# Sartor02/libMultiRobotPlanning

Hardware: AMD Instinct MI355X
Metric: low_level_node_expansions_per_sec (higher is better)
Workload: dtype int32

## Files before the change

### libmultirobotplanning_amd/csrc/ll_jobs.h

```cpp
#ifndef MRP_LL_JOBS_H
#define MRP_LL_JOBS_H

namespace mrp {

__host__ __device__ inline uint32_t ldsBytes(uint32_t pathBytes, bool bg) { return ct::windowBytes(bg) + pathBytes; }

DEVI uint32_t storeLoad(const uint16_t* p) {
#ifdef MRP_LL_STORE_ACQUIRE_FENCE
  return *p;
#else
  return __hip_atomic_load(p, __ATOMIC_RELAXED, __HIP_MEMORY_SCOPE_AGENT);
#endif
}

DEVI uint32_t hostLoad32(const uint32_t* p) { return __hip_atomic_load(p, __ATOMIC_RELAXED, __HIP_MEMORY_SCOPE_SYSTEM); }
DEVI void hostStore32(uint32_t* p, uint32_t v) { __hip_atomic_store(p, v, __ATOMIC_RELAXED, __HIP_MEMORY_SCOPE_SYSTEM); }

DEVI void stageConstraints(const uint32_t* consHost, uint32_t vcOff, uint32_t nVc, uint32_t nEc, uint32_t* consLocal,
                           const uint32_t*& vc, const uint32_t*& ec) {
  const uint32_t* src = consHost + vcOff;
  const uint32_t nWords = nVc + nEc;
  if (nWords <= kConsLocalWords) {
    for (uint32_t i = threadIdx.x; i < nWords; i += 64) consLocal[i] = hostLoad32(src + i);
    vc = consLocal;
  } else {
    __builtin_amdgcn_fence(__ATOMIC_ACQUIRE, "");
    vc = src;
  }
  ec = vc + nVc;
}

__device__ __attribute__((noinline)) bool stageConstraintSet(const DevJob* job, const uint32_t* cons, uint32_t* store, uint32_t stride,
                                                             uint32_t slots, uint32_t* consLocal) {
  const uint32_t nVc = rfl(job->n_vc), nEc = rfl(job->n_ec), dimx = rfl(job->dimx), dimy = rfl(job->dimy);
  const uint32_t baseP1 = rfl(job->pad_[0]), baseCounts = rfl(job->pad_[1]), resP1 = rfl(job->pad_[2]);
  const uint32_t* added = cons + rfl(job->vc_off);
  stride = rfl(stride); slots = rfl(slots);
  const uint32_t bVc = baseP1 ? (baseCounts & 0xFFFFu) : 0u, bEc = baseP1 ? (baseCounts >> 16) : 0u;
  const uint32_t nWords = nVc + nEc;
  if (store == nullptr || baseP1 > slots || resP1 > slots || bVc > nVc || bEc > nEc || nVc > kConsLocalWords ||
      nEc > kConsLocalWords || nWords > kConsLocalWords || nWords > stride)
    return false;
  const uint32_t aVc = nVc - bVc;
  const uint32_t cells = dimx * dimy;
  const uint32_t* base = store + (size_t)(baseP1 ? baseP1 - 1u : 0u) * stride;
  uint32_t* out = store + (size_t)(resP1 ? resP1 - 1u : 0u) * stride;
  for (uint32_t i = threadIdx.x; i < nWords; i += 64) {
    uint32_t w;
    if (i < nVc) {
      if (i < bVc) {
        w = __hip_atomic_load(base + i, __ATOMIC_RELAXED, __HIP_MEMORY_SCOPE_AGENT);
        if ((w & 0xFFu) >= dimx || ((w >> 8) & 0xFFu) >= dimy) w = 0xFFFFFFFFu;
      } else {
        w = hostLoad32(added + (i - bVc));
      }
    } else {
      const uint32_t k = i - nVc;
      if (k < bEc) {
        w = __hip_atomic_load(base + bVc + k, __ATOMIC_RELAXED, __HIP_MEMORY_SCOPE_AGENT);
        if (((w >> 3) & 0xFFFFu) >= cells) w = 0xFFFFFFFFu;
      } else {
        w = hostLoad32(added + aVc + (k - bEc));
      }
    }
    consLocal[i] = w;
    if (resP1) __hip_atomic_store(out + i, w, __ATOMIC_RELAXED, __HIP_MEMORY_SCOPE_AGENT);
  }
  return true;
}

template <bool UNI = false>
DEVI void fillCtx(Ctx& c, const DevJob& J, const uint32_t* maps, volatile uint32_t* debug) {
  auto u = [](uint32_t v) { return UNI ? rfl(v) : v; };
  c.dimx = u(J.dimx); c.dimy = u(J.dimy); c.wpr = u(J.words_per_row);
  c.gx = u(J.gx); c.gy = u(J.gy); c.sx = u(J.sx); c.sy = u(J.sy);
  c.lastGoal = (int32_t)u((uint32_t)J.last_goal_constraint);
  c.w = __builtin_bit_cast(float, u(__builtin_bit_cast(uint32_t, J.w)));
  c.nVc = u(J.n_vc); c.nEc = u(J.n_ec);
  c.obst = maps + u(J.map_word_off);
  c.nAgentsPad = u(J.n_agents_pad); c.tPad = u(J.t_pad);
  c.maxExp = UNI ? (int64_t)rfl64((uint64_t)J.max_expansions) : J.max_expansions;
  c.debug = debug;
}

DEVI void putCJob(uint8_t* smem, const ct::CJob& cj) {
  auto w32 = (__attribute__((address_space(3))) uint32_t*)((wv::Lds)smem + ct::oJob);
  const uint32_t* src = (const uint32_t*)&cj;
#pragma unroll
  for (uint32_t q = 0; q < sizeof(ct::CJob) / 4; ++q) w32[q] = src[q];
}
DEVI ct::CRes getCRes(uint8_t* smem) {
  auto r32 = (__attribute__((address_space(3))) const uint32_t*)((wv::Lds)smem + ct::oRes);
  ct::CRes cr;
  cr.status = (int32_t)rfl(r32[0]); cr.cost = (int32_t)rfl(r32[1]); cr.fmin = (int32_t)rfl(r32[2]);
  cr.nStates = (int32_t)rfl(r32[3]); cr.expanded = rfl(r32[4]); cr.nodes = rfl(r32[5]);
  return cr;
}
DEVI uint32_t narrowOpenCap(const LaunchParams& P) { return P.lds_nodes / 2u < ct::kCap ? P.lds_nodes / 2u : ct::kCap; }
DEVI uint32_t narrowMaxT(const LaunchParams& P) {
  return P.lds_rows >= 3u && P.lds_rows - 2u < ct::kMaxT ? P.lds_rows - 2u : ct::kMaxT;
}
DEVI uint32_t clampMaxExp(int64_t maxExp) {
  return maxExp < 0 ? 0xFFFFFFFFu : (maxExp > 0xFFFFFFFEll ? 0xFFFFFFFEu : (uint32_t)maxExp);
}

DEVI uint8_t* cutHeaps(Mem<TierHbm>& g, uint8_t* p, uint32_t cap) {
  g.open = (Mem<TierHbm>::PE)(p + 8);          p += (size_t)cap * 8 + 16;
  g.focal = (Mem<TierHbm>::PE)(p + 8);         p += (size_t)cap * 8 + 16;
  g.aux = (Mem<TierHbm>::PE)(p + 8);           p += (size_t)cap * 8 + 16;
  g.capNodes = cap; g.capHeap = cap;
  return p;
}
DEVI Mem<TierHbm> cutArena(const LaunchParams& P, uint8_t* arenaSlot) {
  Mem<TierHbm> g = {};
  g.nodes = (Mem<TierHbm>::PN32)arenaSlot;
  g.bits = (Mem<TierHbm>::P32)cutHeaps(g, arenaSlot + slot::nodeBytes(P.arena_nodes), P.arena_nodes);
  g.capRows = P.arena_rows; g.rowWords = P.arena_row_words;
  return g;
}
template <class Geo>
DEVI bool compactFits(uint32_t arenaNodes, uint32_t rows, bool bg) {
  return slot::nodeBytes(arenaNodes) >= Geo::parentBytes(rows) + (bg ? Geo::bitsBytes(rows) : 0u);
}
template <class Geo = ct::Narrow>
DEVI ct::CJob baseCJob(const LaunchParams& P, const DevJob& J, uint8_t* arenaSlot, uint16_t* outPath, uint32_t rows = 0) {
  ct::CJob cj;
  cj.dimx = J.dimx; cj.dimy = J.dimy; cj.w = J.w; cj.obstWords = J.words_per_row;
  cj.obst = (uint64_t)(P.maps + J.map_word_off);
  cj.maxExp = clampMaxExp(J.max_expansions);
  cj.openCap = narrowOpenCap(P); cj.maxT = narrowMaxT(P); cj.taNoGoal = 0; cj.rows = 0;
  cj.parentTab = (uint64_t)arenaSlot; cj.bitsG = (uint64_t)(arenaSlot + Geo::parentBytes(rows)); cj.outPath = (uint64_t)outPath;
  return cj;
}

enum : int { kTiersAll = 0, kTiersFront = 1, kTiersHeavy = 2 };

template <int TIERS>
DEVI bool idTableInLds(const LaunchParams& P, uint32_t pathBytes) {
  return TIERS != kTiersHeavy && P.lds_nodes != 0 && pathBytes <= P.lds_paths_bytes;
}

DEVI bool frontHandsOver(const LaunchParams& P, const DevJob& J) {
  return (J.ctx_flags & kCtxHeavy) != 0 || P.lds_nodes == 0 || J.dimx > 32u || J.dimy > 32u || J.n_agents_pad > 128u || J.n_ec > 64u;
}

DEVI void clearIdTable(uint16_t* dst, uint32_t pathBytes) {
  uint32_t* d32 = (uint32_t*)dst;
  for (uint32_t i = threadIdx.x; i < pathBytes / 4; i += 64) d32[i] = 0xFFFFFFFFu;
#ifdef MRP_LL_STORE_ACQUIRE_FENCE
  __builtin_amdgcn_fence(__ATOMIC_ACQUIRE, "agent");
  asm volatile("s_waitcnt vmcnt(0)" ::: "memory");
#endif
  __syncthreads();
}
DEVI void loadIdChunk(const uint32_t* ids, uint32_t a0, uint32_t nCtx, const uint16_t* store, uint32_t stride, uint32_t slots,
                      uint32_t& idL, uint32_t& lenL) {
  const uint32_t lane = threadIdx.x;
  idL = kNoStoreSlot; lenL = 0;
  if (a0 + lane < nCtx) idL = hostLoad32(ids + a0 + lane);
  if (idL < slots) lenL = storeLoad(store + (size_t)idL * stride);
  if (lenL > stride - 1) lenL = stride - 1;
}
DEVI void buildIdTableInArena(uint16_t* dst, const uint32_t* ids, uint32_t nCtx, uint32_t tPad, uint32_t nAgentsPad,
                              const uint16_t* store, uint32_t stride, uint32_t slots) {
  const uint32_t lane = threadIdx.x;
  clearIdTable(dst, tPad * nAgentsPad * 2);
  for (uint32_t a0 = 0; a0 < nCtx; a0 += 64) {
    uint32_t idL, lenA;
    loadIdChunk(ids, a0, nCtx, store, stride, slots, idL, lenA);
    const uint16_t* slotA = store + (size_t)(idL < slots ? idL : 0) * stride + 1;
    const bool hasA = idL < slots && lenA != 0;
    for (uint32_t t0 = 0; t0 < tPad; t0 += 8) {
      uint32_t v[8];
#pragma unroll
      for (uint32_t u = 0; u < 8; ++u) {
        const uint32_t t = t0 + u;
        v[u] = kEmptyCell;
        if (hasA && t < tPad) v[u] = storeLoad(slotA + (t < lenA ? t : lenA - 1));
      }
#pragma unroll
      for (uint32_t u = 0; u < 8; ++u)
        if (hasA && t0 + u < tPad) dst[(t0 + u) * nAgentsPad + a0 + lane] = (uint16_t)v[u];
    }
  }
}

template <int TIERS>
DEVI bool stageFocalTable(const LaunchParams& P, const DevJob& J, uint8_t* ldsPaths, uint8_t* pathsArena, Ctx& c) {
  constexpr bool kTableMayBeInLds = TIERS != kTiersHeavy;
  const uint32_t lane = threadIdx.x;
  const uint32_t pathBytes = c.tPad * c.nAgentsPad * 2;
  const uint32_t* psrc = (const uint32_t*)(P.paths + J.path_off);
  c.pathsLds = nullptr;
  if (pathBytes != 0 && (J.ctx_flags & kCtxById)) {
    const bool inLds = idTableInLds<TIERS>(P, pathBytes);
    if (!inLds && pathBytes > P.arena_paths_bytes) return false;
    uint16_t* dst = inLds ? (uint16_t*)ldsPaths : (uint16_t*)pathsArena;
    const uint32_t* ids = P.cons + J.path_off;
    const uint32_t nCtx = J.n_ctx;
    if (!inLds) {
      buildIdTableInArena(dst, ids, nCtx, c.tPad, c.nAgentsPad, P.path_store, P.path_store_stride, P.path_store_slots);
    } else {
      clearIdTable(dst, pathBytes);
      for (uint32_t a0 = 0; a0 < nCtx; a0 += 64) {
        uint32_t idL, lenL;
        loadIdChunk(ids, a0, nCtx, P.path_store, P.path_store_stride, P.path_store_slots, idL, lenL);
        const uint32_t nHere = nCtx - a0 < 64 ? nCtx - a0 : 64;
        for (uint32_t t0 = 0; t0 < c.tPad; t0 += 64) {
          const uint32_t t = t0 + lane;
          for (uint32_t q0 = 0; q0 < nHere; q0 += 8) {
            uint32_t v[8];
            bool has[8];
#pragma unroll
            for (uint32_t u = 0; u < 8; ++u) {
              uint32_t id = kNoStoreSlot, len = 0;
              if (q0 + u < nHere) {
                id = __builtin_amdgcn_readlane(idL, q0 + u);
                len = __builtin_amdgcn_readlane(lenL, q0 + u);
              }
              has[u] = id < P.path_store_slots && len != 0 && t < c.tPad;
              v[u] = kEmptyCell;
              if (has[u]) v[u] = storeLoad(P.path_store + (size_t)id * P.path_store_stride + 1 + (t < len ? t : len - 1));
            }
#pragma unroll
            for (uint32_t u = 0; u < 8; ++u)
              if (has[u]) dst[t * c.nAgentsPad + a0 + q0 + u] = (uint16_t)v[u];
          }
        }
      }
    }
    c.paths = dst;
    if (inLds) c.pathsLds = (__attribute__((address_space(3))) const uint16_t*)ldsPaths;
  } else if (pathBytes == 0) {
    c.paths = nullptr;
  } else if (kTableMayBeInLds && P.lds_nodes != 0 && pathBytes <= P.lds_paths_bytes) {
    uint32_t* dst = (uint32_t*)ldsPaths;
    for (uint32_t i = lane; i < pathBytes / 4; i += 64) dst[i] = hostLoad32(psrc + i);
    c.paths = (const uint16_t*)ldsPaths;
    c.pathsLds = (__attribute__((address_space(3))) const uint16_t*)ldsPaths;
  } else if (pathBytes <= P.arena_paths_bytes) {
    uint32_t* dst = (uint32_t*)pathsArena;
    for (uint32_t i = lane; i < pathBytes / 4; i += 64) dst[i] = hostLoad32(psrc + i);
    c.paths = (const uint16_t*)pathsArena;
  } else {
    __builtin_amdgcn_fence(__ATOMIC_ACQUIRE, "");
    c.paths = P.paths + J.path_off;
  }
  return true;
}

template <bool EPS, bool BG, int TIERS, bool TH = false>
DEVI bool compactAttempt(const LaunchParams& P, const DevJob& J, uint8_t* smem, uint8_t* arenaSlot, const Ctx& c, DevResult& res,
                         uint16_t* outPath, SState& s, int& rc, const uint16_t* heur = nullptr) {
  static_assert(!TH || (!BG && TIERS == kTiersAll), "the table form exists for the mixed kernels' narrow tier");
  typedef typename std::conditional<TIERS == kTiersHeavy, ct::Wide, ct::Narrow>::type Geo;
  uint32_t geoRows = Geo::kRows;
  if (TIERS == kTiersHeavy) {
    const uint64_t room = slot::nodeBytes(P.arena_nodes) / (1024u + ct::kRowBytes);
    geoRows = (uint32_t)(room < P.arena_rows ? room : P.arena_rows) & ~63u;
  }
  const bool compactOk = !(TIERS == kTiersAll && (J.ctx_flags & kCtxHeavy) != 0) && P.lds_nodes != 0 && c.dimx <= 32u &&
                         c.dimy <= 32u && c.nAgentsPad <= 128u && c.nEc <= 64u && geoRows >= 64u &&
                         compactFits<Geo>(P.arena_nodes, geoRows, BG) &&
                         (!TH || P.lds_paths_bytes >= 2048u + (EPS && c.pathsLds != nullptr ? c.tPad * c.nAgentsPad * 2u : 0u));
  bool done = false;
  if (compactOk) {
    ct::CJob cj = baseCJob<Geo>(P, J, arenaSlot, outPath, geoRows);
    cj.obstWords = c.wpr;
    cj.sx = c.sx; cj.sy = c.sy; cj.gx = c.gx; cj.gy = c.gy;
    cj.lastGoal = c.lastGoal;
    cj.nVc = c.nVc; cj.nEc = c.nEc;
    cj.nAgentsPad = EPS ? c.nAgentsPad : 0u; cj.tPad = c.tPad;
    cj.rows = geoRows;
    if (TIERS == kTiersHeavy) {
      cj.openCap = Geo::kCap;
      cj.maxT = Geo::kMaxT < geoRows - 2u ? Geo::kMaxT : geoRows - 2u;
    }
    cj.vc = (uint64_t)c.vc; cj.ec = (uint64_t)c.ec;
    cj.pathsG = (uint64_t)c.paths;
    if constexpr (TH) cj.bitsG = (uint64_t)heur;
    putCJob(smem, cj);
    const bool tableInLds = !EPS || c.nAgentsPad == 0u || c.pathsLds != nullptr;
#ifndef MRP_LL_TRACE
    const uint64_t tl0 = __builtin_amdgcn_s_memrealtime();
#endif
    int32_t crc;
    if constexpr (TH && !EPS)
      crc = ct::compactSearch<false, true, false, ct::Narrow, true>((wv::Lds)smem);
    else if constexpr (TH)
      crc = tableInLds ? ct::compactSearch<true, true, false, ct::Narrow, true>((wv::Lds)smem)
                       : ct::compactSearch<true, false, false, ct::Narrow, true>((wv::Lds)smem);
    else if constexpr (TIERS == kTiersHeavy)
      crc = ct::compactSearch<EPS, false, BG, ct::Wide>((wv::Lds)smem);
    else
      crc = tableInLds ? ct::compactSearch<EPS, true, BG>((wv::Lds)smem) : ct::compactSearch<EPS, false, BG>((wv::Lds)smem);
    const ct::CRes cr = getCRes(smem);
#ifndef MRP_LL_TRACE
    res.prof[TIERS == kTiersHeavy ? 2 : 0] = (uint32_t)(__builtin_amdgcn_s_memrealtime() - tl0);
    res.prof[TIERS == kTiersHeavy ? 3 : 1] = cr.expanded;
#endif
#ifdef MRP_CT_PROF
    {
      auto r32 = (__attribute__((address_space(3))) const uint32_t*)((wv::Lds)smem + ct::oRes + 32u);
      for (uint32_t q = 0; q < 8; ++q) res.prof[q] = rfl(r32[q]);
    }
#endif
    if (crc != ct::C_OVERFLOW) {
      rc = crc;
      res.cost = cr.cost; res.fmin = cr.fmin; res.n_states = cr.nStates;
      s.expansions = cr.expanded; s.nNodes = cr.nodes;
      done = true;
      if (TIERS == kTiersHeavy) res.tier = 2;
    } else {
#ifndef MRP_LL_TRACE
      res.prof[6] = cr.expanded;
      res.prof[7] = 1;
#endif
    }
  }
  return done;
}

template <bool EPS, bool BG, int TIERS, bool TH = false>
DEVI int arenaAttempt(const LaunchParams& P, uint8_t* smem, uint8_t* arenaSlot, const Ctx& c, DevResult& res, uint16_t* outPath,
                      SState& s, const uint16_t* heur = nullptr, uint32_t heurStride = 0) {
  typedef typename std::conditional<TIERS == kTiersHeavy, ct::Wide, ct::Narrow>::type Geo;
  int rc;
  const Mem<TierHbm> g = cutArena(P, arenaSlot);
  Mem<TierHyb> gh = viewAs<TierHyb>(g);
  {
    const uint32_t area = Geo::windowBytes(BG) - ct::oOpen;
#ifdef MRP_LL_TOPS_EQUAL
    const uint32_t perO = (area / 3u) & ~15u, perF = perO, perA = perO;
#else
    const uint32_t perO = (area / 2u) & ~15u, perF = (area * 5u / 16u) & ~15u, perA = (area - perO - perF) & ~15u;
#endif
    auto tops = [&](uint32_t per) {
      uint32_t n = per >= 32u ? ((per - 8u) / 8u) : 0u;
      if (n > 4095u) n = 4095u;
      n = n ? ((n - 1u) | 1u) : 0u;
      return P.lds_nodes == 0 ? 0u : n;
    };
    auto l8 = (__attribute__((address_space(3))) uint8_t*)smem + ct::oOpen;
    gh.open = HybPtr{(__attribute__((address_space(3))) uint64_t*)(l8 + 8), (uint64_t*)g.open, tops(perO)};
    gh.focal = HybPtr{(__attribute__((address_space(3))) uint64_t*)(l8 + perO + 8), (uint64_t*)g.focal, tops(perF)};
    gh.aux = HybPtr{(__attribute__((address_space(3))) uint64_t*)(l8 + perO + perF + 8), (uint64_t*)g.aux, tops(perA)};
  }
  const bool xyEntries = P.arena_nodes <= 65536u;
  Mem<TierHybXy> ghx = viewAs<TierHybXy>(gh);
  res.tier = 1;
  __syncthreads();
  if constexpr (TH) {
    if (xyEntries)
      initSearch<TierHybXy, EPS, true>(ghx, s, c, heur, heurStride);
    else
      initSearch<TierHyb, EPS, true>(gh, s, c, heur, heurStride);
  } else if (xyEntries)
    initSearch<TierHybXy, EPS>(ghx, s, c);
  else
    initSearch<TierHyb, EPS>(gh, s, c);
  __syncthreads();
#ifndef MRP_LL_TRACE
  const uint64_t th0 = __builtin_amdgcn_s_memrealtime();
#endif
  if constexpr (TH) {
    if (xyEntries)
      rc = runSearch<TierHybXy, EPS, true>(ghx, s, c, res, outPath, heur, heurStride);
    else
      rc = runSearch<TierHyb, EPS, true>(gh, s, c, res, outPath, heur, heurStride);
  } else if (xyEntries)
    rc = runSearch<TierHybXy, EPS>(ghx, s, c, res, outPath);
  else
    rc = runSearch<TierHyb, EPS>(gh, s, c, res, outPath);
#ifndef MRP_LL_TRACE
  if (TIERS != kTiersHeavy) {
    res.prof[2] = (uint32_t)(__builtin_amdgcn_s_memrealtime() - th0);
    res.prof[3] = (uint32_t)s.expansions;
  }
#endif
  return rc;
}

template <bool EPS, bool BG, int TIERS>
DEVI bool runJob(const LaunchParams& P, const DevJob& J, uint8_t* smem, uint8_t* arenaSlot, DevResult& res,
                 uint16_t* outPath) {
  typedef typename std::conditional<TIERS == kTiersHeavy, ct::Wide, ct::Narrow>::type Geo;
  if (TIERS == kTiersFront && frontHandsOver(P, J)) return true;
  Ctx c;
  fillCtx(c, J, P.maps, P.debug);
  uint32_t* consLocal = slot::consCopy(arenaSlot, P.arena_scratch_off, P.out_stride);
  if ((J.pad_[0] | J.pad_[2]) != 0u) {
    c.vc = consLocal;
    c.ec = consLocal + c.nVc;
  } else {
    stageConstraints(P.cons, J.vc_off, c.nVc, c.nEc, consLocal, c.vc, c.ec);
  }
  if (!stageFocalTable<TIERS>(P, J, smem + Geo::windowBytes(BG), slot::pathsCopy(arenaSlot, P.arena_scratch_off, P.out_stride), c)) {
    res.status = ST_BAD; res.expanded = 0; res.nodes_created = 0;
    return false;
  }
  __syncthreads();
  SState s;
  int rc = ST_BAD;
  res.tier = 0;
  if (!compactAttempt<EPS, BG, TIERS>(P, J, smem, arenaSlot, c, res, outPath, s, rc)) {
    if constexpr (TIERS == kTiersFront)
      return true;
    else
      rc = arenaAttempt<EPS, BG, TIERS>(P, smem, arenaSlot, c, res, outPath, s);
  }
  if (rc == RUN_MIGRATE_NODES) rc = ST_CAP_NODES;
  if (rc == RUN_MIGRATE_ROWS) rc = ST_CAP_HORIZON;
  res.status = rc;
  res.expanded = s.expansions;
  res.nodes_created = s.nNodes;
  return false;
}

template <bool EPS>
__device__ __attribute__((noinline)) void runJobTableH(const DevJob* Jp, DevResult* out, uint8_t* smem, uint8_t* arenaSlot,
                                                       const uint32_t* maps, const uint32_t* consHost, const uint16_t* pathsHost,
                                                       uint32_t scratchOff, uint32_t outStride, uint32_t arenaNodes,
                                                       uint32_t arenaRows, uint32_t arenaRowWords, uint32_t arenaPathsBytes,
                                                       uint32_t ldsNodes, uint32_t ldsPathsBytes) {
  LaunchParams P = {};
  P.maps = (const uint32_t*)rfl64((uint64_t)maps);
  P.cons = (const uint32_t*)rfl64((uint64_t)consHost);
  P.paths = (const uint16_t*)rfl64((uint64_t)pathsHost);
  P.arena_scratch_off = rfl(scratchOff); P.out_stride = rfl(outStride);
  P.arena_nodes = rfl(arenaNodes); P.arena_rows = rfl(arenaRows); P.arena_row_words = rfl(arenaRowWords);
  P.arena_paths_bytes = rfl(arenaPathsBytes);
  P.lds_nodes = rfl(ldsNodes); P.lds_paths_bytes = rfl(ldsPathsBytes);
  smem = (uint8_t*)rfl64((uint64_t)smem);
  arenaSlot = (uint8_t*)rfl64((uint64_t)arenaSlot);
  DevJob J;
  for (uint32_t q = 0; q < sizeof(DevJob) / 4; ++q) ((uint32_t*)&J)[q] = rfl(((const uint32_t*)Jp)[q]);
  J.ctx_flags &= ~kCtxById;
  DevResult res = {};
  Ctx c;
  fillCtx(c, J, P.maps, nullptr);
  if (!EPS) { c.nAgentsPad = 0; c.tPad = 0; }
  uint16_t* outPath = slot::outPath(arenaSlot, P.arena_scratch_off, P.out_stride);
  stageConstraints(P.cons, J.vc_off, c.nVc, c.nEc, slot::consCopy(arenaSlot, P.arena_scratch_off, P.out_stride), c.vc, c.ec);
  {
    LaunchParams Pst = P;
    Pst.lds_paths_bytes = P.lds_paths_bytes >= 2048u ? P.lds_paths_bytes - 2048u : 0u;
    stageFocalTable<kTiersAll>(Pst, J, smem + ct::Narrow::windowBytes(false), slot::pathsCopy(arenaSlot, P.arena_scratch_off, P.out_stride), c);
  }
  __syncthreads();
  const uint16_t* heur = (const uint16_t*)(P.maps + J.heur_off);
  const uint32_t heurStride = (c.dimx <= 32u && c.dimy <= 32u) ? 32u : c.dimx;
  const bool startInMap = c.sx < c.dimx && c.sy < c.dimy;
  const uint32_t h0 = startInMap ? rfl(heur[c.sy * heurStride + c.sx]) : 0u;
  int rc = ST_BAD;
  res.tier = 1;
  if (!startInMap) {
    rc = ST_BAD;
  } else if (h0 == 0xFFFFu) {
    rc = ST_NO_SOLUTION;
  } else if (h0 > kFMax - 2u) {
    rc = ST_CAP_HORIZON;
  } else {
    SState s;
    res.tier = 0;
    if (!compactAttempt<EPS, false, kTiersAll, true>(P, J, smem, arenaSlot, c, res, outPath, s, rc, heur))
      rc = arenaAttempt<EPS, false, kTiersAll, true>(P, smem, arenaSlot, c, res, outPath, s, heur, heurStride);
    if (rc == RUN_MIGRATE_NODES) rc = ST_CAP_NODES;
    if (rc == RUN_MIGRATE_ROWS) rc = ST_CAP_HORIZON;
    res.expanded = s.expansions;
    res.nodes_created = s.nNodes;
  }
  out->status = rc; out->cost = res.cost; out->fmin = res.fmin; out->n_states = res.n_states;
  out->expanded = res.expanded; out->nodes_created = res.nodes_created; out->tier = res.tier;
  for (int q = 0; q < 8; ++q) out->prof[q] = res.prof[q];
}

template <class SidFn>
DEVI void publishPath(const LaunchParams& P, const uint16_t* outPath, uint32_t len, uint32_t* hostDst, SidFn sidOf) {
  const uint32_t lane = threadIdx.x;
  const uint32_t* src = (const uint32_t*)outPath;
  for (uint32_t i = lane; i < (len + 1u) / 2u; i += 64) hostStore32(hostDst + i, src[i]);
  const uint32_t sid = sidOf();
  if (sid < P.path_store_slots && len < P.path_store_stride) {
    uint16_t* slot = P.path_store + (size_t)sid * P.path_store_stride;
    for (uint32_t i = lane; i < len; i += 64) __hip_atomic_store(slot + 1 + i, outPath[i], __ATOMIC_RELAXED, __HIP_MEMORY_SCOPE_AGENT);
    __hip_atomic_store(slot, (uint16_t)len, __ATOMIC_RELAXED, __HIP_MEMORY_SCOPE_AGENT);
  }
}

template <bool HOSTLOADS>
DEVI void beginJob(const DevJob* jobSrc, DevJob& jobS, DevResult& res, uint32_t tier) {
  const uint32_t lane = threadIdx.x;
  const uint32_t* src = (const uint32_t*)jobSrc;
  __syncthreads();
  if (lane < sizeof(DevJob) / 4) ((uint32_t*)&jobS)[lane] = HOSTLOADS ? hostLoad32(src + lane) : src[lane];
  __syncthreads();
  res.status = ST_BAD; res.cost = 0; res.fmin = 0; res.n_states = 0; res.expanded = 0; res.nodes_created = 0;
  res.tier = tier;
  for (int q = 0; q < 8; ++q) res.prof[q] = 0;
}
DEVI void endJob(const DevResult& res, DevResult& resS, DevResult* resDst) {
  __syncthreads();
  resS = res;
  __syncthreads();
  if (threadIdx.x < sizeof(DevResult) / 4) hostStore32((uint32_t*)resDst + threadIdx.x, ((const uint32_t*)&resS)[threadIdx.x]);
}

DEVI void runChain(const LaunchParams& P, const DevJob& J, uint8_t* smem, uint8_t* arenaSlot, DevResult& res,
                   uint16_t* outPath, uint16_t* hostOut) {
  constexpr bool BG = true;
  const uint32_t lane = threadIdx.x;
  const uint32_t n = J.n_ctx, first = J.t_pad, npad = J.n_agents_pad;
  const uint32_t end = J.reserved > first && J.reserved < n ? J.reserved : n;
  res.tier = 0; res.n_states = 0; res.expanded = 0;
  if (P.lds_nodes == 0 || J.dimx > 32u || J.dimy > 32u || n > kChainMaxAgents || first >= n || npad < n || npad > 128u ||
      (npad & 1u) || kChainRows * npad * 2u > (P.lds_paths_bytes != 0u ? P.lds_paths_bytes : P.arena_paths_bytes) ||
      !compactFits<ct::Narrow>(P.arena_nodes, 0, BG) ||
      (uint64_t)n * kChainEntryWords * 2u + (uint64_t)n * 64u > (uint64_t)P.out_host_stride) {
    res.status = ST_BAD;
    return;
  }
  const uint32_t* who = P.cons + J.vc_off;
  const uint32_t* ids = who + n;
  const bool tabInLds = P.lds_paths_bytes != 0u;
  uint16_t* table = (uint16_t*)(tabInLds ? smem + ldsBytes(0, BG) : slot::pathsCopy(arenaSlot, P.arena_scratch_off, P.out_stride));
  for (uint32_t i = lane; i < kChainRows * npad / 2u; i += 64) ((uint32_t*)table)[i] = 0xFFFFFFFFu;
  __syncthreads();
  for (uint32_t a = 0; a < first; ++a) {
    const uint32_t id = rfl(hostLoad32(ids + a));
    if (id >= P.path_store_slots) continue;
    const uint16_t* slot = P.path_store + (size_t)id * P.path_store_stride;
    uint32_t len = rfl(storeLoad(slot));
    if (len > P.path_store_stride - 1) len = P.path_store_stride - 1;
    if (len == 0) continue;
    table[lane * npad + a] = (uint16_t)storeLoad(slot + 1 + (lane < len ? lane : len - 1));
  }
  __syncthreads();
  int64_t budget = J.max_expansions;
  uint32_t* hostW = (uint32_t*)hostOut;
  uint32_t pathOff = n * kChainEntryWords;
  uint32_t done = 0, maxLen = 0;
  bool allOk = true;
  int64_t total = 0;
  for (uint32_t a = first; a < end; ++a) {
    asm volatile("" : "+s"(hostW), "+s"(outPath));
    const uint32_t sg = rfl(hostLoad32(who + a));
    ct::CJob cj = baseCJob(P, J, arenaSlot, outPath);
    cj.sx = sg & 0xFFu; cj.sy = (sg >> 8) & 0xFFu; cj.gx = (sg >> 16) & 0xFFu; cj.gy = sg >> 24;
    cj.lastGoal = -1;
    cj.nVc = 0; cj.nEc = 0;
    cj.nAgentsPad = npad; cj.tPad = kChainRows;
    cj.maxExp = clampMaxExp(budget);
    cj.vc = 0; cj.ec = 0;
    cj.pathsG = tabInLds ? 0ull : (uint64_t)table;
    __syncthreads();
    putCJob(smem, cj);
#ifndef MRP_LL_TRACE
    const uint64_t tl0 = __builtin_amdgcn_s_memrealtime();
#endif
    const int32_t crc = tabInLds ? ct::compactSearch<true, true, BG>((wv::Lds)smem) : ct::compactSearch<true, false, BG>((wv::Lds)smem);
    const ct::CRes cr = getCRes(smem);
    const int32_t cost = cr.cost, fmin = cr.fmin, nStates = cr.nStates;
    const uint32_t expanded = cr.expanded;
#ifndef MRP_LL_TRACE
    res.prof[0] += (uint32_t)(__builtin_amdgcn_s_memrealtime() - tl0);
    res.prof[1] += expanded;
#endif
    if (crc == ct::C_OVERFLOW) {
#ifndef MRP_LL_TRACE
      res.prof[6] += expanded;
      res.prof[7] += 1;
#endif
      allOk = false;
      break;
    }
    {
      uint32_t v = 0;
      v = lane == 0 ? (uint32_t)crc : lane == 1 ? (uint32_t)cost : lane == 2 ? (uint32_t)fmin
          : lane == 3 ? (crc == ct::C_OK ? (uint32_t)nStates : 0u) : lane == 4 ? expanded : lane == 5 ? pathOff : 0u;
      if (lane < kChainEntryWords) hostStore32(hostW + (size_t)done * kChainEntryWords + lane, v);
    }
    done += 1;
    total += expanded;
    if (crc != ct::C_OK) {
      allOk = false;
      break;
    }
    const uint32_t len = (uint32_t)nStates;
    maxLen = len > maxLen ? len : maxLen;
    {
      publishPath(P, outPath, len, hostW + pathOff, [&] { return rfl(hostLoad32(ids + a)); });
      pathOff += (len + 1u) / 2u;
      uint32_t rowLen = npad;
      asm volatile("" : "+s"(rowLen));
      table[lane * rowLen + a] = outPath[lane < len ? lane : len - 1];
    }
    if (budget >= 0) budget = budget > (int64_t)expanded ? budget - (int64_t)expanded : 0;
  }
  __syncthreads();
  res.status = ST_OK;
  res.n_states = (int32_t)done;
  res.expanded = total;
  res.cost = -1;
  res.fmin = -1;
  if (first == 0 && end == n && done == n && allOk && maxLen >= 1u && maxLen <= kChainRows) {
    const uint32_t T = maxLen - 1u;
    uint32_t cnt = 0, key = 0x7FFFFFFFu;
    auto pairsOf = [&](const uint16_t* tab, uint32_t rowC, uint32_t rowN, uint32_t t, bool inT) {
      uint32_t bestV = 0xFFFFu, bestE = 0xFFFFu;
      for (uint32_t i = 0; i + 1u < n; ++i) {
        const uint32_t ci = tab[rowC + i], ni = tab[rowN + i];
        for (uint32_t j = i + 1u; j < n; ++j) {
          const uint32_t cj = tab[rowC + j], nj = tab[rowN + j];
          const bool v = inT && ci == cj, e = inT && ci == nj && ni == cj;
          cnt += (v ? 1u : 0u) + (e ? 1u : 0u);
          if (v && bestV == 0xFFFFu) bestV = (i << 8) | j;
          if (e && bestE == 0xFFFFu) bestE = (i << 8) | j;
        }
      }
      const uint32_t k = bestV != 0xFFFFu ? (t << 24) | bestV : bestE != 0xFFFFu ? (t << 24) | (1u << 16) | bestE : 0x7FFFFFFFu;
      key = k < key ? k : key;
    };
    if (tabInLds) {
      pairsOf(table, lane * npad, (lane + 1u < kChainRows ? lane + 1u : kChainRows - 1u) * npad, lane, lane < T);
    } else {
      uint16_t* stage = (uint16_t*)(smem + ct::oOpen);
      static_assert(2u * ct::kHeapBytes >= 32u * kChainMaxAgents * 2u, "room for 32 rows of the widest table");
      const uint32_t rowsFit = 2u * ct::kHeapBytes / (npad * 2u) < kChainRows ? 2u * ct::kHeapBytes / (npad * 2u) : kChainRows;
      for (uint32_t r0 = 0; r0 < T; r0 += rowsFit - 1u) {
        const uint32_t nRows = kChainRows - r0 < rowsFit ? kChainRows - r0 : rowsFit;
        __syncthreads();
        for (uint32_t i = lane; i < nRows * npad / 2u; i += 64) ((uint32_t*)stage)[i] = ((const uint32_t*)table)[r0 * npad / 2u + i];
        __syncthreads();
        const bool inT = lane + 1u < nRows && r0 + lane < T;
        const uint32_t row = inT ? lane : 0u;
        pairsOf(stage, row * npad, (row + 1u) * npad, r0 + lane, inT);
      }
    }
#pragma unroll
    for (uint32_t off = 32; off >= 1; off >>= 1) {
      cnt += (uint32_t)__shfl_xor((int)cnt, (int)off, 64);
      const uint32_t other = (uint32_t)__shfl_xor((int)key, (int)off, 64);
      key = other < key ? other : key;
    }
    res.cost = (int32_t)rfl(cnt);
    res.fmin = rfl(key) == 0x7FFFFFFFu ? -1 : (int32_t)rfl(key);
  }
}

}

#endif
```

Before: 1.542 billion.

## Stage chain inputs and outputs in device scratch, batch host writes at end

runChain now loads all agent start/goal words and path-store ids from host memory once, in parallel across lanes, into a device-global staging area, and reads them with readlane instead of issuing one system-scope host load per agent. Per-agent result entries and path publication no longer write to host memory inside the sequential search loop. They are collected in the staging area and table and flushed in one batched pass (chainOutput) after the loop. The prefix path loads are also batched 8 at a time to overlap latency. This adds scratch usage and defers host-visible output until chain end, and publication to the path store now happens from the table after the loop.

Measured after the change: 1.513 billion. 0.981x the previous value.

```diff
diff --git a/libmultirobotplanning_amd/csrc/ll_jobs.h b/libmultirobotplanning_amd/csrc/ll_jobs.h
--- a/libmultirobotplanning_amd/csrc/ll_jobs.h
+++ b/libmultirobotplanning_amd/csrc/ll_jobs.h
@@ -153,13 +153,17 @@
 #endif
   __syncthreads();
 }
+DEVI uint32_t idChunkLen(uint32_t idL, const uint16_t* store, uint32_t stride, uint32_t slots) {
+  uint32_t lenL = 0;
+  if (idL < slots) lenL = storeLoad(store + (size_t)idL * stride);
+  return lenL > stride - 1 ? stride - 1 : lenL;
+}
 DEVI void loadIdChunk(const uint32_t* ids, uint32_t a0, uint32_t nCtx, const uint16_t* store, uint32_t stride, uint32_t slots,
                       uint32_t& idL, uint32_t& lenL) {
   const uint32_t lane = threadIdx.x;
-  idL = kNoStoreSlot; lenL = 0;
+  idL = kNoStoreSlot;
   if (a0 + lane < nCtx) idL = hostLoad32(ids + a0 + lane);
-  if (idL < slots) lenL = storeLoad(store + (size_t)idL * stride);
-  if (lenL > stride - 1) lenL = stride - 1;
+  lenL = idChunkLen(idL, store, stride, slots);
 }
 DEVI void buildIdTableInArena(uint16_t* dst, const uint32_t* ids, uint32_t nCtx, uint32_t tPad, uint32_t nAgentsPad,
                               const uint16_t* store, uint32_t stride, uint32_t slots) {
@@ -506,6 +510,50 @@
   if (threadIdx.x < sizeof(DevResult) / 4) hostStore32((uint32_t*)resDst + threadIdx.x, ((const uint32_t*)&resS)[threadIdx.x]);
 }
 
+constexpr uint32_t kChainStageWho = 0, kChainStageIds = kChainMaxAgents, kChainStageEntries = 2u * kChainMaxAgents;
+static_assert(kChainStageEntries + kChainMaxAgents * kChainEntryWords <= kConsLocalWords, "the staging words fit the copy area");
+typedef __attribute__((address_space(1))) uint32_t* ChainStage;
+
+DEVI void chainOutput(const LaunchParams& P, ChainStage stg, const uint16_t* table, uint32_t npad, uint32_t first,
+                      uint32_t done, uint32_t nPaths, uint32_t* hostW) {
+  const uint32_t lane = threadIdx.x;
+  for (uint32_t i = lane; i < done * kChainEntryWords; i += 64) hostStore32(hostW + i, stg[kChainStageEntries + i]);
+  for (uint32_t i0 = 0; i0 < nPaths; i0 += 64) {
+    uint32_t lenL = 0, offL = 0, idL = kNoStoreSlot;
+    if (i0 + lane < nPaths) {
+      const ChainStage e = stg + kChainStageEntries + (i0 + lane) * kChainEntryWords;
+      lenL = e[3]; offL = e[5];
+      idL = stg[kChainStageIds + first + i0 + lane];
+    }
+    if (lenL > kChainRows) lenL = kChainRows;
+    const uint32_t nHere = nPaths - i0 < 64 ? nPaths - i0 : 64;
+    for (uint32_t q0 = 0; q0 < nHere; q0 += 4) {
+      uint32_t c[4], len[4], off[4], sid[4];
+#pragma unroll
+      for (uint32_t u = 0; u < 4; ++u) {
+        len[u] = 0; off[u] = 0; sid[u] = kNoStoreSlot; c[u] = kEmptyCell;
+        if (q0 + u < nHere) {
+          len[u] = __builtin_amdgcn_readlane(lenL, q0 + u);
+          off[u] = __builtin_amdgcn_readlane(offL, q0 + u);
+          sid[u] = __builtin_amdgcn_readlane(idL, q0 + u);
+          c[u] = table[lane * npad + first + i0 + q0 + u];
+        }
+      }
+#pragma unroll
+      for (uint32_t u = 0; u < 4; ++u) {
+        const uint32_t w = (uint32_t)__shfl((int)c[u], (int)((2u * lane) & 63u), 64) |
+                           (uint32_t)__shfl((int)c[u], (int)((2u * lane + 1u) & 63u), 64) << 16;
+        if (lane < (len[u] + 1u) / 2u) hostStore32(hostW + off[u] + lane, w);
+        if (sid[u] < P.path_store_slots && len[u] < P.path_store_stride) {
+          uint16_t* slot = P.path_store + (size_t)sid[u] * P.path_store_stride;
+          if (lane < len[u]) __hip_atomic_store(slot + 1 + lane, (uint16_t)c[u], __ATOMIC_RELAXED, __HIP_MEMORY_SCOPE_AGENT);
+          __hip_atomic_store(slot,(uint16_t)len[u], __ATOMIC_RELAXED, __HIP_MEMORY_SCOPE_AGENT);
+        }
+      }
+    }
+  }
+}
+
 DEVI void runChain(const LaunchParams& P, const DevJob& J, uint8_t* smem, uint8_t* arenaSlot, DevResult& res,
                    uint16_t* outPath, uint16_t* hostOut) {
   constexpr bool BG = true;
@@ -525,26 +573,49 @@
   const bool tabInLds = P.lds_paths_bytes != 0u;
   uint16_t* table = (uint16_t*)(tabInLds ? smem + ldsBytes(0, BG) : slot::pathsCopy(arenaSlot, P.arena_scratch_off, P.out_stride));
   for (uint32_t i = lane; i < kChainRows * npad / 2u; i += 64) ((uint32_t*)table)[i] = 0xFFFFFFFFu;
-  __syncthreads();
-  for (uint32_t a = 0; a < first; ++a) {
-    const uint32_t id = rfl(hostLoad32(ids + a));
-    if (id >= P.path_store_slots) continue;
-    const uint16_t* slot = P.path_store + (size_t)id * P.path_store_stride;
-    uint32_t len = rfl(storeLoad(slot));
-    if (len > P.path_store_stride - 1) len = P.path_store_stride - 1;
-    if (len == 0) continue;
-    table[lane * npad + a] = (uint16_t)storeLoad(slot + 1 + (lane < len ? lane : len - 1));
+  ChainStage stg = (ChainStage)slot::consCopy(arenaSlot, P.arena_scratch_off, P.out_stride);
+  uint32_t idLo = kNoStoreSlot, idHi = kNoStoreSlot;
+  {
+    uint32_t whoLo = 0, whoHi = 0;
+    if (lane < n) { whoLo = hostLoad32(who + lane); idLo = hostLoad32(ids + lane); }
+    if (64u + lane < n) { whoHi = hostLoad32(who + 64u + lane); idHi = hostLoad32(ids + 64u + lane); }
+    stg[kChainStageWho + lane] = whoLo; stg[kChainStageWho + 64u + lane] = whoHi;
+    stg[kChainStageIds + lane] = idLo; stg[kChainStageIds + 64u + lane] = idHi;
+  }
+  __syncthreads();
+  for (uint32_t a0 = 0; a0 < first; a0 += 64) {
+    const uint32_t idL = a0 + lane < first ? (a0 ? idHi : idLo) : kNoStoreSlot;
+    const uint32_t lenL = idChunkLen(idL, P.path_store, P.path_store_stride, P.path_store_slots);
+    const uint32_t nHere = first - a0 < 64 ? first - a0 : 64;
+    for (uint32_t q0 = 0; q0 < nHere; q0 += 8) {
+      uint32_t v[8];
+      bool has[8];
+#pragma unroll
+      for (uint32_t u = 0; u < 8; ++u) {
+        uint32_t id = kNoStoreSlot, len = 0;
+        if (q0 + u < nHere) {
+          id = __builtin_amdgcn_readlane(idL, q0 + u);
+          len = __builtin_amdgcn_readlane(lenL, q0 + u);
+        }
+        has[u] = id < P.path_store_slots && len != 0;
+        v[u] = kEmptyCell;
+        if (has[u]) v[u] = storeLoad(P.path_store + (size_t)id * P.path_store_stride + 1 + (lane < len ? lane : len - 1));
+      }
+#pragma unroll
+      for (uint32_t u = 0; u < 8; ++u)
+        if (has[u]) table[lane * npad + a0 + q0 + u] = (uint16_t)v[u];
+    }
   }
   __syncthreads();
   int64_t budget = J.max_expansions;
   uint32_t* hostW = (uint32_t*)hostOut;
   uint32_t pathOff = n * kChainEntryWords;
-  uint32_t done = 0, maxLen = 0;
+  uint32_t done = 0, nPaths = 0, maxLen = 0;
   bool allOk = true;
   int64_t total = 0;
   for (uint32_t a = first; a < end; ++a) {
-    asm volatile("" : "+s"(hostW), "+s"(outPath));
-    const uint32_t sg = rfl(hostLoad32(who + a));
+    asm volatile("" : "+s"(stg), "+s"(outPath));
+    const uint32_t sg = __builtin_amdgcn_readlane(stg[kChainStageWho + (a & 64u) + lane], a & 63u);
     ct::CJob cj = baseCJob(P, J, arenaSlot, outPath);
     cj.sx = sg & 0xFFu; cj.sy = (sg >> 8) & 0xFFu; cj.gx = (sg >> 16) & 0xFFu; cj.gy = sg >> 24;
     cj.lastGoal = -1;
@@ -578,7 +649,7 @@
       uint32_t v = 0;
       v = lane == 0 ? (uint32_t)crc : lane == 1 ? (uint32_t)cost : lane == 2 ? (uint32_t)fmin
           : lane == 3 ? (crc == ct::C_OK ? (uint32_t)nStates : 0u) : lane == 4 ? expanded : lane == 5 ? pathOff : 0u;
-      if (lane < kChainEntryWords) hostStore32(hostW + (size_t)done * kChainEntryWords + lane, v);
+      if (lane < kChainEntryWords) stg[kChainStageEntries + done * kChainEntryWords + lane] = v;
     }
     done += 1;
     total += expanded;
@@ -589,7 +660,7 @@
     const uint32_t len = (uint32_t)nStates;
     maxLen = len > maxLen ? len : maxLen;
     {
-      publishPath(P, outPath, len, hostW + pathOff, [&] { return rfl(hostLoad32(ids + a)); });
+      nPaths += 1;
       pathOff += (len + 1u) / 2u;
       uint32_t rowLen = npad;
       asm volatile("" : "+s"(rowLen));
@@ -646,8 +717,9 @@
     res.cost = (int32_t)rfl(cnt);
     res.fmin = rfl(key) == 0x7FFFFFFFu ? -1 : (int32_t)rfl(key);
   }
-}
-
-}
-
-#endif
+  chainOutput(P, stg, table, npad, first, done, nPaths, hostW);
+}
+
+}
+
+#endif
```
